# Vinmwaura/Quantized-Autoregression-Image-Generator

Hardware: AMD Instinct MI355X
Metric: image-tokens/sec at 1/2/4/8 GPUs; BMU argmin GB/s vs HBM peak (higher is better)
Workload: dtype f32; 1 GPU; BASELINE configs[1]: BMU (K=512; LR patch 32, HR patch 2) + base decoder-only Transformer train step, 32x32x4 latents (128x128 images), 257-token sequences, window 256; batch_per_gpu=64, global_batch=64, seq_len=256, in_dim=512, hidden_dim=2048, heads=64, dec_layers=7, enc_layers=0, params=78226440, parallelism=dp1, launch=eager stream launches

## Files before the change

include/qarig.h:

```cpp
#ifndef QARIG_H
#define QARIG_H

#include <stddef.h>
#include <stdint.h>

#ifdef __cplusplus
extern "C" {
#endif

#define QARIG_OK 0
#define QARIG_ERR_ARG -1
#define QARIG_ERR_LAUNCH -2
#define QARIG_ERR_WORKSPACE -3

#define QARIG_ACT_NONE 0
#define QARIG_ACT_SILU 1
#define QARIG_ACT_TANH 2
#define QARIG_ACT_SIGMOID 3

int qarig_version(void);
const char* qarig_target_arch(void);
int qarig_last_error(char* buf, size_t n);
int qarig_set_option(const char* name, int value);

// ... 150 lines not shown

int qarig_window_step_supported(int R, int window, int D, int H);

int qarig_window_assemble(const int64_t* ring, int64_t ldr, const int* ctl, int R, int W1, int Wp, int D,
                          int V, const float* table, const float* pe, int P, int pos_off, float* x,
                          int* rowmap, int* last_map, int* bad_flag, void* stream);

int qarig_window_attention(const float* q, const float* k, const float* v, int R, int H, int d, int n_keys,
                           int rows, int64_t batch_stride, const float* o_mul, int64_t ldmul, float* o,
                           void* stream);

int qarig_window_append(int* ctl, const int64_t* ids, int64_t* ring, int B, int64_t ldr, int* bad_flag,
                        void* stream);

size_t qarig_colsum_workspace_bytes(int M, int N);
int qarig_colsum_f32(const float* X, int64_t ldx, int M, int N, float* out, int accumulate,
                     void* workspace, size_t ws_bytes, void* stream);

int qarig_slab_reduce_rowsum_f32(const float* slabs, float* out, int64_t ldc, int M, int N, int nslab,
                                 int accumulate, const float* rs_part, float* rs_out, void* stream);


int qarig_patchify_fwd(const float* image, int N, int C, int H, int W, int pH, int pW,
                       float* patches, void* stream);
int qarig_unpatchify_fwd(const float* patches, int N, int C, int H, int W, int pH, int pW,
                         float* image, void* stream);

int qarig_codebook_gather_image(const int64_t* ids, int N, int C, int H, int W, int pH, int pW,
                                const float* codebook, int K, float* image, int* bad_flag,
                                void* stream);

int qarig_gather_rows(const int64_t* ids, int64_t R, int D, int K, const float* table, float* out,
                      int* bad_flag, void* stream);

int qarig_som_weights_fwd(const int64_t* bmu, int64_t R, int K, float two_var, float* g,
                          void* stream);

int qarig_som_band(const float* in, int K, int D, float two_var, int reach, float* out, void* stream);

int qarig_index_histogram(const int64_t* ids, int64_t n, int K, int64_t* counts, int* bad_flag,
                          void* stream);


int qarig_posemb_fwd(const float* pos, int R, int D, const float* freq, float* out, void* stream);

int qarig_assemble_tokens(const int64_t* lr, int S_lr, const int64_t* hr, int S_hr, int N, int base,
                          int k_lr, int k_hr, const int64_t* offs, int W, int64_t* hr_in,
                          int64_t* hr_tg, int64_t* pos, int* bad_flag, void* stream);

int qarig_embedding_fwd(const int64_t* ids, int M, int S, int D, int V, const float* table,
                        const float* pe, float* out, int* bad_flag, void* stream);
int qarig_embedding_bwd(const int64_t* ids, int M, int D, int V, const float* dy, float* dtable,
                        void* stream);

int qarig_layernorm_fwd(const float* x, int M, int D, float eps, const float* gamma,
                        const float* beta, const float* scale, const float* shift,
                        const int* mod_idx, float* y, float* mean, float* rstd, void* stream);
int qarig_layernorm_bwd(const float* dy, const float* x, const float* mean, const float* rstd,
                        const float* gamma, const float* scale, const int* mod_idx, int M, int D,
                        float* dx, float* dy_xhat, const float* dx_add, void* stream);

int qarig_rowmap_build(const int* idx, int M, int P, int* counts, int* offsets, int* rows,
                       int* bad_flag, void* stream);
int qarig_segment_sum(const float* src, const int* offsets, const int* rows, int P, int D,
                      float* out, void* stream);
int qarig_mul_rows_fwd(const float* a, const float* tab, const int* idx, float* y, int M, int D,
                       void* stream);
int qarig_mul_rows_bwd(const float* dy, const float* a, const float* tab, const int* idx, float* da,
                       float* db_tok, int M, int D, void* stream);
int qarig_layernorm_bwd_table(const float* dy, const float* x, const float* mean, const float* rstd,
                              const float* scale_tab, const int* offsets, const int* rows, int M, int P,
                              int D, float* dx, const float* dx_add, float* dscale, float* dshift,
                              void* stream);
int qarig_mul_rows_bwd_table(const float* dy, const float* a, const float* tab, const int* offsets,
                             const int* rows, int M, int P, int D, float* da, float* dg, void* stream);

int qarig_attention_fwd(const float* q, const float* k, const float* v, int N, int Sq, int Sk,
                        int H, int d, int causal, float sqrt_d, float* o, float* lse,
                        void* stream);
int qarig_attention_bwd(const float* q, const float* k, const float* v, const float* o,
                        const float* dO, const float* lse, int N, int Sq, int Sk, int H, int d,
                        int causal, float sqrt_d, float* dq, float* dk, float* dv, float* delta,
                        void* stream);

int qarig_attention_lp_fwd(const float* q, const float* k, const float* v, int N, int Sq, int Sk, int H,
                           int d, int causal, float sqrt_d, float* o, float* lse, void* stream);
int qarig_attention_lp_bwd(const float* q, const float* k, const float* v, const float* o,
                           const float* dO, const float* lse, int N, int Sq, int Sk, int H, int d,
                           int causal, float sqrt_d, float* dq, float* dk, float* dv, float* delta,
                           void* stream);

int qarig_attention_decode(const float* q, const float* k_new, const float* v_new, float* kcache,
                           float* vcache, int B, int H, int d, int len, const int* len_dev,
                           int max_len, int64_t batch_stride, float sqrt_d, const float* o_mul,
                           float* o, void* stream);

int qarig_cross_entropy_fwd(const float* logits, const int64_t* target, int M, int C, float* loss,
                            float* dlogits, float* row_ws, int* bad_flag, void* stream);
int qarig_cross_entropy_ld_fwd(const float* logits, int64_t ld_logits, const int64_t* target, int M, int C,
                               float* loss, float* dlogits, int64_t ld_dlogits, float* row_ws, int* bad_flag,
                               void* stream);

int qarig_cross_entropy_reg_fwd(const float* logits, const int64_t* target, int M, int C, float label_smoothing,
                                float z_loss, float* loss, float* dlogits, float* row_ws, int* bad_flag,
                                void* stream);

int qarig_token_score(const float* logits, const int64_t* target, int M, int C, int64_t ignore_index,
                      float* row_nll, int* row_rank, int* bad_flag, void* stream);
int qarig_score_reduce(const float* row_nll, const int* row_rank, int N, int S, int pos0, int P, int topk,
                       double* img_nll, double* pos_nll, int64_t* pos_cnt, int64_t* totals, void* stream);

size_t qarig_pair_error_workspace_bytes(int N, int64_t E);
int qarig_pair_error(const float* a, const float* b, int N, int64_t E, double* out, void* ws, size_t ws_bytes,
                     void* stream);
size_t qarig_ssim_workspace_bytes(int N, int C, int H, int W, int taps);
int qarig_ssim(const float* a, const float* b, int N, int C, int H, int W, const double* win, int taps, double c1,
               double c2, double* out, void* ws, size_t ws_bytes, void* stream);

size_t qarig_ssim_maps_bytes(int N, int C, int H, int W, int taps);
int qarig_ssim_fwd_maps(const float* a, const float* b, int N, int C, int H, int W, const double* win, int taps,
                        double c1, double c2, double* out, double* maps, void* ws, size_t ws_bytes, void* stream);
int qarig_ssim_bwd(const float* a, const float* b, const double* maps, const double* g, int N, int C, int H, int W,
                   const double* win, int taps, float* da, void* stream);

size_t qarig_mse_workspace_bytes(void);
int qarig_mse_fwd(const float* pred, const float* target, int64_t n, float* loss, float* dpred,
                  float* part_ws, void* stream);

int qarig_adam_step(float* p, const float* g, float* m, float* v, int64_t n, float beta1,
                    float beta2, float eps, float step_size, float bc2_sqrt, float grad_scale,
                    const float* dev_step, void* shadow_bf16, void* stream);

int qarig_adam_ema_step(float* p, const float* g, float* m, float* v, float* ema, int64_t n, float beta1,
                        float beta2, float eps, float step_size, float bc2_sqrt, float ema_w,
                        float grad_scale, const float* dev_step, void* shadow_bf16, void* stream);

int qarig_adamw_step(float* p, const float* g, float* m, float* v, float* ema, const unsigned char* decay_mask,
                     int64_t n, float beta1, float beta2, float eps, float step_size, float bc2_sqrt,
                     float ema_w, float decay, float grad_scale, const float* dev_step, void* shadow_bf16,
                     void* stream);

#define QARIG_GRAD_NORM_PARTIALS 2048
int qarig_grad_clip_coef(const float* g, int64_t n, float grad_scale, double max_norm, double* partials,
                         double* state, void* stream);
int qarig_adam_clip_step(float* p, const float* g, float* m, float* v, float* ema, const unsigned char* decay_mask,
                         int64_t n, float beta1, float beta2, float eps, float step_size, float bc2_sqrt,
                         float ema_w, float decay, float grad_scale, const float* dev_step, void* shadow_bf16,
                         const double* clip_state, void* stream);

int qarig_swap_f32(float* a, float* b, int64_t n, void* stream);

int qarig_mul_fwd(const float* a, const float* b, float* y, int64_t n, void* stream);
int qarig_mul_bwd(const float* dy, const float* a, const float* b, float* da, float* db, int64_t n,
                  void* stream);
int qarig_act_fwd(const float* x, float* y, int64_t n, int act, void* stream);
int qarig_act_bwd(const float* dy, const float* z, float* dz, int64_t n, int act, void* stream);
int qarig_scale_by(const float* x, const float* s, float* y, int64_t n, void* stream);

int qarig_dropout(const float* x, float* y, int64_t n, uint32_t threshold, float scale, uint32_t site,
                  const uint32_t* key, void* stream);


int qarig_conv2d_fwd(const float* x, int N, int Cin, int H, int W, const float* w,
                     const float* bias, int Cout, int k, int stride, int pad, int act, float* y,
                     float* preact, void* stream);
size_t qarig_conv2d_fwd_workspace_bytes(int Cin, int Cout, int k);
// ... 33 lines not shown
```

quantized-autoregression-image-generator_amd/csrc/attention.hip:

```cpp
#include <stdlib.h>

#include "qarig_common.h"

namespace qarig {

struct AttnDims {
    int N, Sq, Sk, H, causal;
    float c2;
    float rsd;
};

__device__ __forceinline__ float exp2_fast(float x) { return __builtin_amdgcn_exp2f(x); }

constexpr int HPB = 4;

__device__ __forceinline__ f32x4 mfma4(float a, float b, f32x4 c) {
    return __builtin_amdgcn_mfma_f32_4x4x1f32(a, b, c, 0, 0, 0);
}

typedef short s16x4 __attribute__((ext_vector_type(4)));
__device__ __forceinline__ uint32_t pack2_bf16(float a, float b) {
    typedef __bf16 bf16x2_t __attribute__((ext_vector_type(2)));
    typedef float f32x2_t __attribute__((ext_vector_type(2)));
    const f32x2_t f = {a, b};
// ... 442 lines not shown
        if (ibeg > c0) i0 = c0 + ((ibeg - c0) & ~7);
        for (; i0 < i1; i0 += 8) {
            const int ii = i0 - c0;
            f32x4 s0 = {0.f, 0.f, 0.f, 0.f}, s1 = s0, d0 = s0, d1 = s0;
            const T* qr = Qc + (ii + li) * Geo<HD>::RS;
            const T* gr = Gc + (ii + li) * Geo<HD>::RS;
            dot_rows<LP, HD>(s0, qr, kv);
            dot_rows<LP, HD>(s1, qr + 4 * Geo<HD>::RS, kv);
            dot_rows<LP, HD>(d0, gr, vv);
            dot_rows<LP, HD>(d1, gr + 4 * Geo<HD>::RS, vv);
            const f32x4 La = *reinterpret_cast<const f32x4*>(Lc + ii);
            const f32x4 Lb = *reinterpret_cast<const f32x4*>(Lc + ii + 4);
            const f32x4 Da = *reinterpret_cast<const f32x4*>(Dc + ii);
            const f32x4 Db = *reinterpret_cast<const f32x4*>(Dc + ii + 4);
            float p[8], ds[8];
#pragma unroll
            for (int r = 0; r < 4; ++r) {
                p[r] = exp2_fast(fmaf(s0[r], a.c2, -La[r]));
                p[4 + r] = exp2_fast(fmaf(s1[r], a.c2, -Lb[r]));
            }
            if (i0 + 8 > i1 || (a.causal && i0 < k0 + 63)) {
#pragma unroll
                for (int r = 0; r < 8; ++r)
                    if (i0 + r >= i1 || (a.causal && j > i0 + r)) p[r] = 0.0f;
            }
#pragma unroll
            for (int r = 0; r < 4; ++r) {
                ds[r] = p[r] * (d0[r] - Da[r]);
                ds[4 + r] = p[4 + r] * (d1[r] - Db[r]);
            }
            const Vals<LP> pa = make_vals<LP>(p[0], p[1], p[2], p[3]);
            const Vals<LP> pb = make_vals<LP>(p[4], p[5], p[6], p[7]);
            const Vals<LP> da = make_vals<LP>(ds[0], ds[1], ds[2], ds[3]);
            const Vals<LP> dbv = make_vals<LP>(ds[4], ds[5], ds[6], ds[7]);
#pragma unroll
            for (int g = 0; g < G; ++g) {
                const T* gt = GTc + (4 * g + li) * TS + ii;
                const T* qt = QTc + (4 * g + li) * TS + ii;
                if constexpr (LP) {
                    acc_cols<LP>(dva[g], gt, pa);
                    acc_cols<LP>(dka[g], qt, da);
                    acc_cols<LP>(dva[g], gt + 4, pb);
                    acc_cols<LP>(dka[g], qt + 4, dbv);
                } else {
                    const f32x4 ga = *reinterpret_cast<const f32x4*>(gt);
                    const f32x4 gb4 = *reinterpret_cast<const f32x4*>(gt + 4);
                    const f32x4 qa = *reinterpret_cast<const f32x4*>(qt);
                    const f32x4 qb4 = *reinterpret_cast<const f32x4*>(qt + 4);
#pragma unroll
                    for (int r = 0; r < 4; ++r) {
                        dva[g] = mfma4(ga[r], p[r], dva[g]);
                        dka[g] = mfma4(qa[r], ds[r], dka[g]);
                    }
#pragma unroll
                    for (int r = 0; r < 4; ++r) {
                        dva[g] = mfma4(gb4[r], p[4 + r], dva[g]);
                        dka[g] = mfma4(qb4[r], ds[4 + r], dka[g]);
                    }
                }
            }
        }
        if (t + 1 < nchunks) {
            T* nb = smem + ((t + 1) & 1) * BUF;
            chunk_store_rows<HD>(nb, rq);
            chunk_store_rows<HD>(nb + GOFF, rg);
            chunk_store_transposed<HD>(nb + QTOFF, TS, rq);
            chunk_store_transposed<HD>(nb + GTOFF, TS, rg);
            float* nl = ldbase + ((t + 1) & 1) * LDBUF;
            if (lth) { nl[threadIdx.x] = rl; nl[HPB * CH + threadIdx.x] = rd; }
        }
        __syncthreads();
    }
    if (active) {
#pragma unroll
        for (int g = 0; g < G; ++g) {
            *reinterpret_cast<float4*>(dk + roff + 4 * g) =
                make_float4(dka[g][0] * a.rsd, dka[g][1] * a.rsd, dka[g][2] * a.rsd, dka[g][3] * a.rsd);
            *reinterpret_cast<float4*>(dv + roff + 4 * g) =
                make_float4(dva[g][0], dva[g][1], dva[g][2], dva[g][3]);
        }
    }
}


}

using namespace qarig;

#define QARIG_HD_DISPATCH(d, ...)                                              \
    switch (d) {                                                                 \
        case 4: { constexpr int HD = 4; __VA_ARGS__; } break;                           \
        case 8: { constexpr int HD = 8; __VA_ARGS__; } break;                           \
        case 16: { constexpr int HD = 16; __VA_ARGS__; } break;                         \
        case 32: { constexpr int HD = 32; __VA_ARGS__; } break;                         \
        case 64: { constexpr int HD = 64; __VA_ARGS__; } break;                         \
        default:                                                                 \
            qarig_set_error("attention: head dim %d unsupported (4,8,16,32,64,128)", d); \
            return QARIG_ERR_ARG;                                                \
    }

int qarig_attention_wide_fwd(const float* q, const float* k, const float* v, int N, int Sq, int Sk, int H,
                             int causal, float sqrt_d, float* o, float* lse, hipStream_t st);
int qarig_attention_wide_bwd(const float* q, const float* k, const float* v, const float* o, const float* dO,
                             const float* lse, int N, int Sq, int Sk, int H, int causal, float sqrt_d, float* dq,
                             float* dk, float* dv, float* delta, hipStream_t st);
static int attn_wide_check(int N, int Sq, int Sk, int H, int causal) {
    QARIG_CHECK_ARG(N > 0 && Sq > 0 && Sk > 0 && H > 0, "attention: bad extents");
    QARIG_CHECK_DIMS("attention", N, Sq, H);
    QARIG_CHECK_DIMS("attention", N, Sk, H);
    QARIG_CHECK_ARG(H <= 65535 && N <= 65535, "attention (wide heads): more than 65535 heads or sequences");
    QARIG_CHECK_ARG(!causal || Sq == Sk, "attention: causal needs Sq == Sk (self-attention)");
    return QARIG_OK;
}

static int attn_check(int N, int Sq, int Sk, int H, int d, int causal) {
    QARIG_CHECK_ARG(N > 0 && Sq > 0 && Sk > 0 && H > 0 && d > 0, "attention: bad extents");
    QARIG_CHECK_DIMS("attention", N, Sq, H);
    QARIG_CHECK_DIMS("attention", N, Sk, H);
    QARIG_CHECK_ARG(d == 4 || d == 8 || d == 16 || d == 32 || d == 64,
                    "attention: head dim %d unsupported (4,8,16,32,64,128)", d);
    QARIG_CHECK_ARG((long long)N * ((H + 3) / 4) * ((Sq > Sk ? Sq : Sk) / 64 + 1) < (1LL << 31),
                    "attention: too many workgroups");
    QARIG_CHECK_ARG(!causal || Sq == Sk, "attention: causal needs Sq == Sk (self-attention)");
    return QARIG_OK;
}

static int attn_waves(int rows, int d, int option, int dflt, int wmax) {
    int w = option > 0 ? option : dflt;
    w = w >= 4 ? 4 : (w >= 2 ? 2 : 1);
    if (w > wmax) w = wmax;
    while (w > 1 && (w / 2) * 64 >= rows) w /= 2;
    while (w < wmax && (w * 256) / d < 8) w *= 2;
    return w;
}

#define QARIG_FWD_MAXT(HD) ((HD) <= 16 ? 1024 : 512)

template <typename K>
static int attn_set_lds(K kernel, size_t bytes, const char* what) {
    if (bytes > 160 * 1024) {
        qarig_set_error("%s: needs %zu B of LDS", what, bytes);
        return QARIG_ERR_ARG;
    }
    if (bytes > 48 * 1024) {
        hipError_t e = hipFuncSetAttribute(reinterpret_cast<const void*>(kernel),
                                           hipFuncAttributeMaxDynamicSharedMemorySize, (int)bytes);
        if (e != hipSuccess) {
            qarig_set_error("%s: hipFuncSetAttribute(%zu B LDS): %s", what, bytes, hipGetErrorString(e));
            return QARIG_ERR_LAUNCH;
        }
    }
    return QARIG_OK;
}

static size_t attn_lds_bytes(int threads, int d, int rows, int tr, bool ld, int lp) {
    const int W = HPB * d, CH = threads / (W / 4);
    const size_t img = 2 * (lp ? 2 : 4) * ((size_t)rows * CH * (W + 4) + (size_t)tr * W * (CH + 4));
    return ((img + 15) & ~(size_t)15) + (ld ? 2 * sizeof(float) * 2 * HPB * CH : 0);
}

template <bool LP>
static int attention_fwd_impl(const float* q, const float* k, const float* v, int N, int Sq, int Sk,
                              int H, int d, int causal, float sqrt_d, float* o, float* lse, void* stream) {
    QARIG_CHECK_ARG(q && k && v && o && lse, "attention_fwd: null pointer");
    if (d == 128) {
        if (int e = attn_wide_check(N, Sq, Sk, H, causal)) return e;
        QARIG_CHECK_ARG(sqrt_d > 0.0f, "attention: sqrt_d must be positive");
        return qarig_attention_wide_fwd(q, k, v, N, Sq, Sk, H, causal, sqrt_d, o, lse, (hipStream_t)stream);
    }
    if (int e = attn_check(N, Sq, Sk, H, d, causal)) return e;
    AttnDims a{N, Sq, Sk, H, causal, 1.4426950408889634f / sqrt_d, 1.0f / sqrt_d};
    const int W = attn_waves(Sq, d, g_qarig_opt.attn_qw, 2, d <= 16 ? 4 : 2);
    const int threads = 256 * W, rows = 64 * W;
    const size_t lds = attn_lds_bytes(threads, d, 1, 1, false, LP);
    dim3 grid((unsigned)(N * ((H + HPB - 1) / HPB) * ((Sq + rows - 1) / rows))), block(threads);
    QARIG_HD_DISPATCH(d, {
        auto kern = attn_fwd_kernel<HD, QARIG_FWD_MAXT(HD), LP>;
        if (int e = attn_set_lds(kern, lds, "attention_fwd")) return e;
        hipLaunchKernelGGL(kern, grid, block, lds, (hipStream_t)stream, q, k, v, a, o, lse);
    });
    QARIG_CHECK_LAUNCH("attention_fwd");
    return QARIG_OK;
}

template <bool LP>
static int attention_bwd_impl(const float* q, const float* k, const float* v, const float* o,
                              const float* dO, const float* lse, int N, int Sq, int Sk, int H, int d,
                              int causal, float sqrt_d, float* dq, float* dk, float* dv, float* delta,
                              void* stream) {
    QARIG_CHECK_ARG(q && k && v && o && dO && lse && dq && dk && dv && delta,
                    "attention_bwd: null pointer");
    if (d == 128) {
        if (int e = attn_wide_check(N, Sq, Sk, H, causal)) return e;
        QARIG_CHECK_ARG(sqrt_d > 0.0f, "attention: sqrt_d must be positive");
        return qarig_attention_wide_bwd(q, k, v, o, dO, lse, N, Sq, Sk, H, causal, sqrt_d, dq, dk, dv, delta,
                                        (hipStream_t)stream);
    }
    if (int e = attn_check(N, Sq, Sk, H, d, causal)) return e;
    AttnDims a{N, Sq, Sk, H, causal, 1.4426950408889634f / sqrt_d, 1.0f / sqrt_d};
    const int hgroups = (H + HPB - 1) / HPB;
    {
        const int W = attn_waves(Sq, d, g_qarig_opt.attn_bw, 2, 2);
        const int threads = 256 * W, rows = 64 * W;
        const size_t lds = attn_lds_bytes(threads, d, 2, 1, false, LP);
        dim3 grid((unsigned)(N * hgroups * ((Sq + rows - 1) / rows))), block(threads);
        QARIG_HD_DISPATCH(d, {
            auto kern = attn_bwd_dq_kernel<HD, 512, LP>;
            if (int e = attn_set_lds(kern, lds, "attention_bwd dq")) return e;
            hipLaunchKernelGGL(kern, grid, block, lds, (hipStream_t)stream, q, k, v, o, dO, lse, a, dq, delta);
        });
        QARIG_CHECK_LAUNCH("attention_bwd dq");
    }
    {
        const int W = attn_waves(Sk, d, g_qarig_opt.attn_bw, 2, 2);
        const int threads = 256 * W, rows = 64 * W;
        const size_t lds = attn_lds_bytes(threads, d, 2, 2, true, LP);
        dim3 grid((unsigned)(N * hgroups * ((Sk + rows - 1) / rows))), block(threads);
        QARIG_HD_DISPATCH(d, {
            auto kern = attn_bwd_dkv_kernel<HD, 512, LP>;
            if (int e = attn_set_lds(kern, lds, "attention_bwd dkv")) return e;
            hipLaunchKernelGGL(kern, grid, block, lds, (hipStream_t)stream, q, k, v, dO, lse, delta, a, dk, dv);
        });
        QARIG_CHECK_LAUNCH("attention_bwd dkv");
    }
    return QARIG_OK;
}

extern "C" int qarig_attention_fwd(const float* q, const float* k, const float* v, int N, int Sq,
                                   int Sk, int H, int d, int causal, float sqrt_d, float* o,
                                   float* lse, void* stream) {
    return attention_fwd_impl<false>(q, k, v, N, Sq, Sk, H, d, causal, sqrt_d, o, lse, stream);
}

extern "C" int qarig_attention_bwd(const float* q, const float* k, const float* v, const float* o,
                                   const float* dO, const float* lse, int N, int Sq, int Sk, int H,
                                   int d, int causal, float sqrt_d, float* dq, float* dk, float* dv,
                                   float* delta, void* stream) {
    return attention_bwd_impl<false>(q, k, v, o, dO, lse, N, Sq, Sk, H, d, causal, sqrt_d, dq, dk, dv,
                                     delta, stream);
}

extern "C" int qarig_attention_lp_fwd(const float* q, const float* k, const float* v, int N, int Sq,
                                      int Sk, int H, int d, int causal, float sqrt_d, float* o,
                                      float* lse, void* stream) {
    return attention_fwd_impl<true>(q, k, v, N, Sq, Sk, H, d, causal, sqrt_d, o, lse, stream);
}
extern "C" int qarig_attention_lp_bwd(const float* q, const float* k, const float* v, const float* o,
                                      const float* dO, const float* lse, int N, int Sq, int Sk, int H,
                                      int d, int causal, float sqrt_d, float* dq, float* dk, float* dv,
                                      float* delta, void* stream) {
    return attention_bwd_impl<true>(q, k, v, o, dO, lse, N, Sq, Sk, H, d, causal, sqrt_d, dq, dk, dv,
                                    delta, stream);
}

extern "C" int qarig_attention_decode(const float* q, const float* k_new, const float* v_new,
                                      float* kcache, float* vcache, int B, int H, int d, int len,
                                      const int* len_dev, int max_len, int64_t batch_stride,
                                      float sqrt_d, const float* o_mul, float* o, void* stream) {
    return qarig_decode_attention(q, k_new, v_new, kcache, vcache, B, H, d, len, len_dev, max_len, batch_stride, d,
                                  (int64_t)H * d, sqrt_d, o_mul, (int64_t)H * d, o, stream);
}
```

quantized-autoregression-image-generator_amd/csrc/capi.hip:

```cpp
#include <stdarg.h>
#include <stdio.h>
#include <string.h>

#include "qarig_common.h"

static thread_local char g_err[512] = "";

extern "C" void qarig_set_error(const char* fmt, ...) {
    va_list ap;
    va_start(ap, fmt);
    vsnprintf(g_err, sizeof(g_err), fmt, ap);
    va_end(ap);
}

extern "C" int qarig_version(void) { return 100; }

extern "C" int qarig_last_error(char* buf, size_t n) {
    if (!buf || n == 0) return QARIG_ERR_ARG;
    strncpy(buf, g_err, n - 1);
    buf[n - 1] = '\0';
    return QARIG_OK;
}

extern "C" const char* qarig_target_arch(void) { return "gfx950"; }

QarigOptions g_qarig_opt;

extern "C" int qarig_set_option(const char* name, int value) {
    struct Entry { const char* name; int* slot; };
    const Entry table[] = {
        {"gemm_dma", &g_qarig_opt.gemm_dma},       {"gemm_pair", &g_qarig_opt.gemm_pair},
        {"bmu_cs", &g_qarig_opt.bmu_cs},           {"bmu_groups", &g_qarig_opt.bmu_groups},
        {"bmu_coarse", &g_qarig_opt.bmu_coarse},   {"attn_qw", &g_qarig_opt.attn_qw},
        {"attn_bw", &g_qarig_opt.attn_bw},         {"lp_big", &g_qarig_opt.lp_big},
        {"lp_mfma16", &g_qarig_opt.lp_mfma16},     {"convt_pair", &g_qarig_opt.convt_pair},
        {"conv_ring", &g_qarig_opt.conv_ring},     {"gemm_xcd_splits", &g_qarig_opt.gemm_xcd_splits},
        {"decode_stream", &g_qarig_opt.decode_stream}, {"decode_rows", &g_qarig_opt.decode_rows},
        {"gemm_tile64", &g_qarig_opt.gemm_tile64}, {"gemm_x3", &g_qarig_opt.gemm_x3},
    };
    if (name)
        for (const Entry& e : table)
            if (strcmp(e.name, name) == 0) {
                const int old = *e.slot;
                *e.slot = value;
                return old;
            }
    qarig_set_error("set_option: unknown option %s (gemm_dma, gemm_pair, bmu_cs, bmu_groups, bmu_coarse, attn_qw, "
                    "attn_bw, lp_big, lp_mfma16, convt_pair, conv_ring, gemm_xcd_splits, decode_stream, decode_rows, gemm_tile64, gemm_x3)", name ? name : "(null)");
    return -2147483647 - 1;
}
```

quantized-autoregression-image-generator_amd/csrc/qarig_common.h:

```cpp
#pragma once
#include <hip/hip_runtime.h>
#include <stdint.h>

#define QARIG_OK 0
#define QARIG_ERR_ARG -1
#define QARIG_ERR_LAUNCH -2
#define QARIG_ERR_WORKSPACE -3

extern "C" void qarig_set_error(const char* fmt, ...);

extern "C" int qarig_gemm_tile64(int M, int N, int K);
extern "C" int qarig_decode_linear_supported(int M, int N, int K, int ln);
extern "C" int qarig_decode_linear_f32(const float* X, int64_t ldx, int64_t x_gs, float eps, const float* gamma,
                                       const float* beta, const float* scale, const float* shift, int64_t ldmod,
                                       const float* W, int64_t ldw, int64_t w_gs, const float* bias, int64_t bias_gs,
                                       const float* residual, int64_t ldr, const float* mul, int64_t ldmul, float* C,
                                       int64_t ldc, int64_t c_gs, int groups, int M, int N, int K, int act,
                                       void* stream);
extern "C" int qarig_decode_attention(const float* q, const float* k_new, const float* v_new, float* kcache,
                                      float* vcache, int B, int H, int d, int len, const int* len_dev, int max_len,
                                      int64_t batch_stride, int64_t head_stride, int64_t row_stride, float sqrt_d,
                                      const float* o_mul, int64_t ldmul, float* o, void* stream);

struct QarigOptions {
    int gemm_dma = 1;
    int gemm_xcd_splits = 1;
    int gemm_pair = -1;
    int bmu_cs = 0;
    int bmu_groups = -1;
    int bmu_coarse = -1;
    int attn_qw = 0;
    int attn_bw = 0;
    int lp_big = -1;
    int lp_mfma16 = 1;
    int convt_pair = 1;
    int gemm_x3 = 0;
    int gemm_tile64 = -1;
    int decode_rows = 1;
    int decode_stream = 1;
    int conv_ring = 1;
};
extern QarigOptions g_qarig_opt;

#define QARIG_CHECK_ARG(cond, ...)                 \
    do {                                           \
        if (!(cond)) {                             \
            qarig_set_error(__VA_ARGS__);          \
            return QARIG_ERR_ARG;                  \
        }                                          \
    } while (0)

#define QARIG_CHECK_LAUNCH(name)                                              \
    do {                                                                      \
        hipError_t e__ = hipGetLastError();                                   \
        if (e__ != hipSuccess) {                                              \
            qarig_set_error("%s: launch failed: %s", name, hipGetErrorString(e__)); \
            return QARIG_ERR_LAUNCH;                                          \
        }                                                                     \
    } while (0)

#include <initializer_list>
static inline bool qarig_dims_ok(std::initializer_list<long long> dims, long long max_each = 1LL << 24,
                                 long long max_prod = 1LL << 40) {
    long long p = 1;
    for (long long d : dims) {
        if (d < 1 || d > max_each) return false;
        if (p > max_prod / d) return false;
        p *= d;
    }
    return true;
}
#define QARIG_CHECK_DIMS(what, ...)                                                             \
    QARIG_CHECK_ARG(qarig_dims_ok({__VA_ARGS__}),                                               \
                    what ": extents must be positive, at most 2^24 each, product at most 2^40")

namespace qarig {

typedef float f32x16 __attribute__((ext_vector_type(16)));
typedef float f32x4 __attribute__((ext_vector_type(4)));

enum Act : int { ACT_NONE = 0, ACT_SILU = 1, ACT_TANH = 2, ACT_SIGMOID = 3 };

__device__ __forceinline__ float sigmoid_f(float x) {
    return __builtin_amdgcn_rcpf(1.0f + __builtin_amdgcn_exp2f(x * -1.4426950408889634f));
}

__device__ __forceinline__ float act_fwd(float x, int act) {
    switch (act) {
        case ACT_SILU: return x * sigmoid_f(x);
        case ACT_TANH: return tanhf(x);
        case ACT_SIGMOID: return sigmoid_f(x);
        default: return x;
    }
}

__device__ __forceinline__ float act_grad(float x, int act) {
    switch (act) {
        case ACT_SILU: {
            float s = sigmoid_f(x);
            return s * (1.0f + x * (1.0f - s));
        }
        case ACT_TANH: {
            float t = tanhf(x);
            return 1.0f - t * t;
        }
        case ACT_SIGMOID: {
            float s = sigmoid_f(x);
            return s * (1.0f - s);
        }
        default: return 1.0f;
    }
}

constexpr int BM = 128;
constexpr int BN = 128;
// ... 266 lines not shown
```

quantized-autoregression-image-generator_amd/qarig/_lib.py:

```python
import ctypes
import os
from ctypes import c_int, c_int64, c_size_t, c_void_p, c_float, c_char_p

import torch

_HERE = os.path.dirname(os.path.abspath(__file__))
LIB_PATH = os.path.join(os.path.dirname(_HERE), "lib",
                        os.environ.get("QARIG_LIB", "libqarig_hip.so"))

P = c_void_p
I = c_int
L = c_int64
Z = c_size_t
F = c_float
D = ctypes.c_double
U = ctypes.c_uint32

SIGNATURES = {
    "qarig_version": (I, []),
    "qarig_target_arch": (c_char_p, []),
    "qarig_last_error": (I, [c_char_p, Z]),
    "qarig_set_option": (I, [c_char_p, I]),
    "qarig_bmu_workspace_bytes": (Z, [L, I]),
    "qarig_bmu_fwd": (I, [P, I, I, I, I, I, I, P, I, I, P, P, Z, P]),
    "qarig_bmu_fwd_prepared": (I, [P, I, I, I, I, I, I, P, I, I, P, P, Z, P, P]),
    "qarig_bmu_fwd_coarse": (I, [P, I, I, I, I, I, I, P, I, I, P, P, P, P]),
    "qarig_bmu_coarse_workspace_bytes": (Z, [L, I]),
    "qarig_bmu_fwd_coarse_ws": (I, [P, I, I, I, I, I, I, P, I, I, P, P, P, P, Z, P]),
    "qarig_bmu_prepare_bytes": (Z, [I, I]),
    "qarig_bmu_prepare": (I, [P, I, I, P, P]),
    "qarig_gemm_ragged_tn": (I, [I, I, I]),
    "qarig_gemm_ragged_nt": (I, [I, I, I]),
    "qarig_gemm_workspace_bytes": (Z, [I, I, I]),
    "qarig_gemm_f32": (I, [P, L, I, P, L, I, P, L, I, I, I, P, P, L, P, L, I, P, L, I, I, I, P, P, Z,
                           P]),
    "qarig_gemm_tile64": (I, [I, I, I]),
    "qarig_gemm_x3_ok": (I, [I, I, I, I]),
    "qarig_gemm_grouped_supported": (I, [I, I, I, I]),
    "qarig_gemm_grouped_workspace_bytes": (Z, [I, I, I, I, I]),
    "qarig_gemm_f32_grouped": (I, [I, P, L, I, P, L, I, P, L, I, I, I, P, P, L, P, L, I, P, L, I, I, I, I, P,
                                   P, Z, P]),
    "qarig_gemm_f32_strided": (I, [P, L, P, L, L, P, L, L, P, L, I, I, I, I, I, P]),
    "qarig_gemm_lp_supported": (I, [I, I, I, I]),
    "qarig_gemm_lp_workspace_bytes": (Z, [I, I, I]),
    "qarig_gemm_lp": (I, [P, L, P, L, I, P, L, I, I, I, P, P, L, P, L, I, P, L, I, I, I, I, P, L, P, L, P, Z,
                          P]),
    "qarig_gemm_f8_supported": (I, [I, I, I]),
    "qarig_cast_fp8": (I, [P, L, P, P, P, P, P]),
    "qarig_gemm_f8": (I, [P, L, P, L, P, P, P, L, I, I, I, P, P, L, P, L, I, P, L, P, L, P]),
    "qarig_mx_quant_workspace_bytes": (Z, [I, I]),
    "qarig_mx_quant": (I, [P, L, I, I, I, P, P, P, P, P, I, P, Z, P]),
    "qarig_gemm_mx_supported": (I, [I, I, I, I]),
    "qarig_gemm_mx_workspace_bytes": (Z, [I, I, I]),
    "qarig_gemm_mx": (I, [P, L, P, L, P, L, P, L, P, L, I, I, I, P, P, L, P, L, I, P, L, I, I, I, I, P, L, P, L,
                          P, Z, P]),
    "qarig_cast_colsum_workspace_bytes": (Z, [I, I]),
    "qarig_cast_colsum": (I, [P, L, I, I, I, P, P, I, P, Z, P]),
    "qarig_cast_bf16": (I, [P, P, L, P]),
    "qarig_cast_transpose_bf16": (I, [P, L, I, I, P, P]),
    "qarig_colsum_workspace_bytes": (Z, [I, I]),
    "qarig_colsum_f32": (I, [P, L, I, I, P, I, P, Z, P]),
    "qarig_patchify_fwd": (I, [P, I, I, I, I, I, I, P, P]),
    "qarig_unpatchify_fwd": (I, [P, I, I, I, I, I, I, P, P]),
    "qarig_codebook_gather_image": (I, [P, I, I, I, I, I, I, P, I, P, P, P]),
    "qarig_gather_rows": (I, [P, L, I, I, P, P, P, P]),
    "qarig_som_weights_fwd": (I, [P, L, I, F, P, P]),
    "qarig_som_band": (I, [P, I, I, F, I, P, P]),
    "qarig_index_histogram": (I, [P, L, I, P, P, P]),
    "qarig_posemb_fwd": (I, [P, I, I, P, P, P]),
    "qarig_assemble_tokens": (I, [P, I, P, I, I, I, I, I, P, I, P, P, P, P, P]),
    "qarig_embedding_fwd": (I, [P, I, I, I, I, P, P, P, P, P]),
    "qarig_embedding_bwd": (I, [P, I, I, I, P, P, P]),
    "qarig_layernorm_fwd": (I, [P, I, I, F, P, P, P, P, P, P, P, P, P]),
    "qarig_layernorm_bwd": (I, [P, P, P, P, P, P, P, I, I, P, P, P, P]),
    "qarig_rowmap_build": (I, [P, I, I, P, P, P, P, P]),
    "qarig_segment_sum": (I, [P, P, P, I, I, P, P]),
    "qarig_mul_rows_fwd": (I, [P, P, P, P, I, I, P]),
    "qarig_mul_rows_bwd": (I, [P, P, P, P, P, P, I, I, P]),
    "qarig_layernorm_bwd_table": (I, [P, P, P, P, P, P, P, I, I, I, P, P, P, P, P]),
    "qarig_mul_rows_bwd_table": (I, [P, P, P, P, P, I, I, I, P, P, P]),
    "qarig_slab_reduce_rowsum_f32": (I, [P, P, L, I, I, I, I, P, P, P]),
    "qarig_attention_fwd": (I, [P, P, P, I, I, I, I, I, I, F, P, P, P]),
    "qarig_attention_lp_fwd": (I, [P, P, P, I, I, I, I, I, I, F, P, P, P]),
    "qarig_attention_lp_bwd": (I, [P, P, P, P, P, P, I, I, I, I, I, I, F, P, P, P, P, P]),
    "qarig_attention_decode": (I, [P, P, P, P, P, I, I, I, I, P, I, L, F, P, P, P]),
    "qarig_gemm_grouped_skinny_f32": (I, [P, L, L, P, L, L, P, L, L, P, L, I, I, I, I, I, P]),
    "qarig_gemm_skinny_ln_f32": (I, [P, L, F, P, P, P, P, L, P, L, L, P, L, L, P, L, P, L, I, I, I, I, I, P]),
    "qarig_decode_linear_supported": (I, [I, I, I, I]),
    "qarig_decode_linear_f32": (I, [P, L, L, F, P, P, P, P, L, P, L, L, P, L, P, L, P, L, P, L, L, I, I, I, I, I,
                                    P]),
    "qarig_decode_linear_bf16w": (I, [P, L, L, F, P, P, P, P, L, P, L, L, P, L, P, L, P, L, P, L, L, I, I, I, I, I,
                                      P]),
    "qarig_decode_embed": (I, [P, I, I, I, P, P, P, I, I, P, L, P, P, P, P]),
    "qarig_decode_attention_keys_per_pass": (ctypes.c_uint, [I]),
    "qarig_decode_attention": (I, [P, P, P, P, P, I, I, I, I, P, I, L, L, L, F, P, L, P, P]),
    "qarig_decode_sample": (I, [P, L, I, I, F, I, I, L, P, P, P, I, I, I, I, I, P, P, P, P, P]),
    "qarig_decode_sample_filtered": (I, [P, L, I, I, F, I, I, L, P, P, P, I, I, I, I, I, P, P, P, P, I, F, P]),
    "qarig_decode_decide": (I, [P, I, I, I, I, P, P, P, P, P, P]),
    "qarig_decode_rows": (I, [P, P, P, P, I, I, I, I, I, I, I, I, P]),
    "qarig_decode_cache_fill": (I, [P, P, L, L, P, I, I, I, I, I, I, P]),
    "qarig_decode_commit": (I, [P, I, I, I, P, P, L, P, P]),
    "qarig_decode_advance": (I, [P, I, P]),
    "qarig_window_step_supported": (I, [I, I, I, I]),
    "qarig_window_assemble": (I, [P, L, P, I, I, I, I, I, P, P, I, I, P, P, P, P, P]),
    "qarig_window_attention": (I, [P, P, P, I, I, I, I, I, L, P, L, P, P]),
    "qarig_window_append": (I, [P, P, P, I, L, P, P]),
    "qarig_attention_bwd": (I, [P, P, P, P, P, P, I, I, I, I, I, I, F, P, P, P, P, P]),
    "qarig_cross_entropy_fwd": (I, [P, P, I, I, P, P, P, P, P]),
    "qarig_cross_entropy_ld_fwd": (I, [P, L, P, I, I, P, P, L, P, P, P]),
    "qarig_cross_entropy_reg_fwd": (I, [P, P, I, I, F, F, P, P, P, P, P]),
    "qarig_token_score": (I, [P, P, I, I, L, P, P, P, P]),
    "qarig_score_reduce": (I, [P, P, I, I, I, I, I, P, P, P, P, P]),
    "qarig_pair_error_workspace_bytes": (Z, [I, L]),
    "qarig_pair_error": (I, [P, P, I, L, P, P, Z, P]),
    "qarig_ssim_workspace_bytes": (Z, [I, I, I, I, I]),
    "qarig_ssim": (I, [P, P, I, I, I, I, P, I, D, D, P, P, Z, P]),
    "qarig_ssim_maps_bytes": (Z, [I, I, I, I, I]),
    "qarig_ssim_fwd_maps": (I, [P, P, I, I, I, I, P, I, D, D, P, P, P, Z, P]),
    "qarig_ssim_bwd": (I, [P, P, P, P, I, I, I, I, P, I, P, P]),
    "qarig_mse_workspace_bytes": (Z, []),
    "qarig_mse_fwd": (I, [P, P, L, P, P, P, P]),
    "qarig_adam_step": (I, [P, P, P, P, L, F, F, F, F, F, F, P, P, P]),
    "qarig_adam_ema_step": (I, [P, P, P, P, P, L, F, F, F, F, F, F, F, P, P, P]),
    "qarig_adamw_step": (I, [P, P, P, P, P, P, L, F, F, F, F, F, F, F, F, P, P, P]),
    "qarig_grad_clip_coef": (I, [P, L, F, D, P, P, P]),
    "qarig_adam_clip_step": (I, [P, P, P, P, P, P, L, F, F, F, F, F, F, F, F, P, P, P, P]),
    "qarig_swap_f32": (I, [P, P, L, P]),
    "qarig_mul_fwd": (I, [P, P, P, L, P]),
    "qarig_mul_bwd": (I, [P, P, P, P, P, L, P]),
    "qarig_act_fwd": (I, [P, P, L, I, P]),
    "qarig_act_bwd": (I, [P, P, P, L, I, P]),
    "qarig_scale_by": (I, [P, P, P, L, P]),
    "qarig_dropout": (I, [P, P, L, U, F, U, P, P]),
    "qarig_conv2d_fwd": (I, [P, I, I, I, I, P, P, I, I, I, I, I, P, P, P]),
    "qarig_conv2d_fwd_workspace_bytes": (Z, [I, I, I]),
    "qarig_conv2d_fwd_workspace_bytes_n": (Z, [I, I, I, I, I, I, I]),
    "qarig_conv2d_fwd_ws": (I, [P, I, I, I, I, P, P, I, I, I, I, I, P, P, P, Z, I, P]),
    "qarig_conv_transpose2d_workspace_bytes": (Z, [I, I]),
    "qarig_conv_transpose2d_workspace_bytes_n": (Z, [I, I, I, I, I]),
    "qarig_conv_transpose2d_fwd": (I, [P, I, I, I, I, P, P, I, I, P, P, P, Z, I, P]),
    "qarig_conv2d_bwd_data_workspace_bytes": (Z, [I, I, I]),
    "qarig_conv2d_bwd_data_workspace_bytes_n": (Z, [I, I, I, I, I, I, I]),
    "qarig_conv_transpose2d_bwd_data_workspace_bytes_n": (Z, [I, I, I, I, I]),
    "qarig_conv2d_bwd_data": (I, [P, I, I, I, I, P, I, I, I, I, I, I, P, P, Z, P]),
    "qarig_conv_transpose2d_bwd_data": (I, [P, I, I, I, I, P, I, P, P]),
    "qarig_conv_transpose2d_bwd_data_ws": (I, [P, I, I, I, I, P, I, P, P, Z, P]),
    "qarig_conv_wgrad_workspace_bytes": (Z, [I, I, I]),
    "qarig_conv_wgrad": (I, [P, I, I, I, I, P, I, I, I, I, I, I, P, P, Z, P]),
    "qarig_conv_bias_grad": (I, [P, I, I, I, P, P]),
}

_lib = None


def load():
    global _lib
    if _lib is not None:
        return _lib
    if not os.path.exists(LIB_PATH):
        raise RuntimeError(
            f"{LIB_PATH} not found: build it with "
            "`python quantized-autoregression-image-generator_amd/build.py` "
            "(there is no CPU fallback for the qarig ops)")
    lib = ctypes.CDLL(LIB_PATH)
    for name, (res, args) in SIGNATURES.items():
        fn = getattr(lib, name)
        fn.restype = res
        fn.argtypes = args
    _lib = lib
    for name in OPTIONS:
        v = os.environ.get("QARIG_" + name.upper())
        if v is not None:
            lib.qarig_set_option(name.encode(), int(v))
            _option_values[name] = int(v)
    return lib


OPTIONS = ("gemm_dma", "gemm_pair", "bmu_cs", "bmu_groups", "bmu_coarse", "attn_qw", "attn_bw", "lp_big",
           "lp_mfma16", "convt_pair", "conv_ring", "gemm_xcd_splits", "decode_stream", "decode_rows", "gemm_tile64", "gemm_x3")


OPTION_EPOCH = 0


_option_values = {}


def set_option(name, value):
    global OPTION_EPOCH
    OPTION_EPOCH += 1
    old = load().qarig_set_option(name.encode(), int(value))
    if old == -2 ** 31:
        raise KeyError(f"{name}: {last_error()}")
    _option_values[name] = int(value)
    return old


def option_value(name):
    return _option_values.get(name)


def last_error():
    buf = ctypes.create_string_buffer(512)
    load().qarig_last_error(buf, 512)
    return buf.value.decode("utf-8", "replace")


N_CALLS = 0


def check(status, what):
    global N_CALLS
    N_CALLS += 1
    if status != 0:
        raise RuntimeError(f"{what} failed ({status}): {last_error()}")


def ptr(t):
    if t is None:
        return None
    return t.data_ptr()


_raw_stream = getattr(torch._C, "_cuda_getCurrentRawStream", None)


def stream():
    if _raw_stream is not None:
        return _raw_stream(torch.cuda.current_device())
    return torch.cuda.current_stream().cuda_stream


def require_cuda(*tensors):
    for t in tensors:
        if t is not None and not t.is_cuda:
            raise RuntimeError(
                "qarig ops run on MI355X only: got a CPU tensor "
                "(the CPU restatement lives in oracle/ and is test infrastructure)")


def f32c(t):
    if t.dtype != torch.float32:
        t = t.float()
    return t if t.is_contiguous() else t.contiguous()


_ws_cache = {}
_ws_retired = []


def workspace(nbytes, device, tag="default"):
    key = (device.index if device.index is not None else torch.cuda.current_device(), tag)
    buf = _ws_cache.get(key)
    if buf is None or buf.numel() < nbytes:
        if buf is not None:
            _ws_retired.append(buf)
        buf = torch.empty(max(int(nbytes), 1 << 20), dtype=torch.uint8, device=device)
        _ws_cache[key] = buf
    return buf
```

Before: 294,900 image-tokens/s.

## Add single-pass attention backward kernel for head dim 8 with LDS-accumulated dq

Adds a fused attention backward kernel for head dim 8 and sequences up to 256. Each block keeps dq accumulators for the whole sequence in LDS per wave and computes dk, dv and dq in one sweep over query chunks, replacing the previous multi-pass or multi-kernel backward. It is meant to cut redundant recomputation and global traffic for dq. The cost is a large LDS footprint, which may lower occupancy. A plan function and an option are added to gate the path.

```diff
diff --git a/include/qarig.h b/include/qarig.h
--- a/include/qarig.h
+++ b/include/qarig.h
@@ -256,6 +256,7 @@
                         const float* dO, const float* lse, int N, int Sq, int Sk, int H, int d,
                         int causal, float sqrt_d, float* dq, float* dk, float* dv, float* delta,
                         void* stream);
+int qarig_attention_bwd_plan(int Sq, int Sk, int H, int d, int causal, int lp);
 
 int qarig_attention_lp_fwd(const float* q, const float* k, const float* v, int N, int Sq, int Sk, int H,
                            int d, int causal, float sqrt_d, float* o, float* lse, void* stream);
diff --git a/quantized-autoregression-image-generator_amd/csrc/attention.hip b/quantized-autoregression-image-generator_amd/csrc/attention.hip
--- a/quantized-autoregression-image-generator_amd/csrc/attention.hip
+++ b/quantized-autoregression-image-generator_amd/csrc/attention.hip
@@ -548,6 +548,263 @@
     }
 }
 
+constexpr int ONEPASS_MAX_S = 256;
+constexpr int OP_ROUND = 16;
+constexpr int OP_TS = 64 + 4;
+constexpr int op_chunk(int kw) { return 32 * kw; }
+constexpr int op_shared(int kw) {
+    return 2 * op_chunk(kw) * (HPB * 8 + 4) + 2 * HPB * 8 * (op_chunk(kw) + 4) + 2 * HPB * op_chunk(kw);
+}
+constexpr int OP_WAVE = OP_ROUND * OP_TS + ONEPASS_MAX_S * 8;
+
+__device__ __forceinline__ void wave_lds_sync() {
+    __builtin_amdgcn_fence(__ATOMIC_RELEASE, "wavefront");
+    __builtin_amdgcn_wave_barrier();
+    __builtin_amdgcn_fence(__ATOMIC_ACQUIRE, "wavefront");
+}
+
+template <bool B> struct BoolC { static constexpr bool value = B; };
+
+template <int HD, int KW>
+__global__ __launch_bounds__(256 * KW, 2) void attn_bwd_onepass_kernel(
+    const float* __restrict__ q, const float* __restrict__ k, const float* __restrict__ v,
+    const float* __restrict__ o, const float* __restrict__ dO, const float* __restrict__ lse, AttnDims a,
+    float* __restrict__ dq, float* __restrict__ dk, float* __restrict__ dv) {
+    static_assert(HD == 8, "the lane = (key half, query, column group) mapping is that of two column groups");
+    static_assert(KW == 1 || KW == 2, "one or two waves per head");
+    extern __shared__ __attribute__((aligned(16))) unsigned char smem_raw[];
+    float* smem = reinterpret_cast<float*>(smem_raw);
+    constexpr int G = HD / 4;
+    constexpr int CH = op_chunk(KW), TS = CH + 4, RS = Geo<HD>::RS, W = Geo<HD>::W;
+    constexpr int GOFF = CH * RS, QTOFF = 2 * CH * RS, GTOFF = QTOFF + W * TS;
+    constexpr int LOFF = GTOFF + W * TS, DOFF = LOFF + HPB * CH;
+    constexpr int OP_SHARED = op_shared(KW);
+    static_assert(DOFF + HPB * CH == OP_SHARED, "LDS layout");
+    const int hgroups = (a.H + HPB - 1) / HPB;
+    const int hg = blockIdx.x % hgroups, n = blockIdx.x / hgroups;
+    const int lane = threadIdx.x & 63;
+    const int wave = __builtin_amdgcn_readfirstlane(threadIdx.x >> 6);
+    const int hh = wave & 3, kh = wave >> 2;
+    const int h = hg * HPB + hh;
+    const bool head_ok = h < a.H;
+    const int D = a.H * HD;
+    const int li = lane & 3;
+    const int cols_valid = (a.H - hg * HPB) * HD;
+    const int ks = lane >> 5, g2 = (lane >> 2) & 1, qrow = ((lane >> 3) & 3) * 4 + li;
+    float* tile = smem + OP_SHARED + wave * OP_WAVE;
+    float* accq = tile + OP_ROUND * OP_TS;
+#pragma unroll
+    for (int m = 0; m < ONEPASS_MAX_S * HD / 256; ++m)
+        *reinterpret_cast<f32x4*>(accq + (m * 64 + lane) * 4) = f32x4{0.f, 0.f, 0.f, 0.f};
+    const float* Qc = smem + hh * HD;
+    const float* Gc = smem + GOFF + hh * HD;
+    const float* QTc = smem + QTOFF + (hh * HD) * TS;
+    const float* GTc = smem + GTOFF + (hh * HD) * TS;
+    const float* Lc = smem + LOFF + hh * CH;
+    const float* Dc = smem + DOFF + hh * CH;
+
+    const float* qbase = q + (int64_t)n * a.Sq * D + hg * HPB * HD;
+    const float* gbase = dO + (int64_t)n * a.Sq * D + hg * HPB * HD;
+    const float* obase = o + (int64_t)n * a.Sq * D + hg * HPB * HD;
+    const float* lb = lse + ((int64_t)n * a.H + hg * HPB) * a.Sq;
+    const int lrow = threadIdx.x / CH, lcol = threadIdx.x - lrow * CH;
+    const bool lth = threadIdx.x < HPB * CH;
+    auto load_ld = [&](int c0, float& rl, float& rd) {
+        rl = 0.0f; rd = 0.0f;
+        if (lth && hg * HPB + lrow < a.H && c0 + lcol < a.Sq) {
+            rl = lb[(int64_t)lrow * a.Sq + c0 + lcol];
+            const int64_t ro = (int64_t)(c0 + lcol) * D + lrow * HD;
+#pragma unroll
+            for (int c = 0; c < HD; c += 4) {
+                const float4 tg = *reinterpret_cast<const float4*>(gbase + ro + c);
+                const float4 to = *reinterpret_cast<const float4*>(obase + ro + c);
+                rd = fmaf(tg.x, to.x, rd); rd = fmaf(tg.y, to.y, rd);
+                rd = fmaf(tg.z, to.z, rd); rd = fmaf(tg.w, to.w, rd);
+            }
+        }
+    };
+
+    const int nkg = (a.Sk + 63) >> 6;
+    const int nslots = KW == 1 ? nkg : (nkg > 2 ? 2 : 1);
+    for (int slot = 0; slot < nslots; ++slot) {
+        const int kg = KW == 1 ? slot : (slot == 0 ? kh : 3 - kh);
+        const bool part = kg < nkg;
+        const int k0 = kg * 64;
+        const int j = k0 + lane;
+        const bool active = part && head_ok && j < a.Sk;
+        const int64_t roff = ((int64_t)n * a.Sk + (active ? j : 0)) * D + h * HD;
+        Own<false, HD> kv, vv;
+        own_load<false, HD>(kv, k + roff, active);
+        own_load<false, HD>(vv, v + roff, active);
+        float kt[32];
+        wave_lds_sync();
+#pragma unroll
+        for (int c = 0; c < HD; ++c) tile[c * OP_TS + lane] = kv.f[c];
+        wave_lds_sync();
+#pragma unroll
+        for (int m = 0; m < 8; ++m) {
+            const f32x4 t4 = *reinterpret_cast<const f32x4*>(tile + (4 * g2 + li) * OP_TS + 32 * ks + 4 * m);
+            kt[4 * m] = t4[0]; kt[4 * m + 1] = t4[1]; kt[4 * m + 2] = t4[2]; kt[4 * m + 3] = t4[3];
+        }
+        wave_lds_sync();
+        f32x4 dka[G], dva[G];
+#pragma unroll
+        for (int g = 0; g < G; ++g) { dka[g] = f32x4{0.f, 0.f, 0.f, 0.f}; dva[g] = dka[g]; }
+
+        const int ibeg = !a.causal ? 0 : (KW == 1 ? k0 : 128 * slot);
+        const int nchunks = a.Sq > ibeg ? (a.Sq - ibeg + CH - 1) / CH : 0;
+        const int qlo = j >= a.Sk ? 0x7fffffff : (a.causal ? j : 0);
+
+        auto round = [&](int i0, int c0, int i1, auto edge_c) {
+            constexpr bool EDGE = decltype(edge_c)::value;
+#pragma unroll
+            for (int st = 0; st < OP_ROUND / 8; ++st) {
+                const int is = i0 + 8 * st, ii = is - c0;
+                const float* qr = Qc + (ii + li) * RS;
+                const float* gr = Gc + (ii + li) * RS;
+                f32x4 qa[G], qb[G], ga[G], gb[G];
+#pragma unroll
+                for (int g = 0; g < G; ++g) {
+                    qa[g] = *reinterpret_cast<const f32x4*>(qr + 4 * g);
+                    qb[g] = *reinterpret_cast<const f32x4*>(qr + 4 * RS + 4 * g);
+                    ga[g] = *reinterpret_cast<const f32x4*>(gr + 4 * g);
+                    gb[g] = *reinterpret_cast<const f32x4*>(gr + 4 * RS + 4 * g);
+                }
+                const f32x4 La = *reinterpret_cast<const f32x4*>(Lc + ii);
+                const f32x4 Lb = *reinterpret_cast<const f32x4*>(Lc + ii + 4);
+                const f32x4 Da = *reinterpret_cast<const f32x4*>(Dc + ii);
+                const f32x4 Db = *reinterpret_cast<const f32x4*>(Dc + ii + 4);
+                f32x4 gta[G], gtb[G], qta[G], qtb[G];
+#pragma unroll
+                for (int g = 0; g < G; ++g) {
+                    const float* gt = GTc + (4 * g + li) * TS + ii;
+                    const float* qt = QTc + (4 * g + li) * TS + ii;
+                    gta[g] = *reinterpret_cast<const f32x4*>(gt);
+                    gtb[g] = *reinterpret_cast<const f32x4*>(gt + 4);
+                    qta[g] = *reinterpret_cast<const f32x4*>(qt);
+                    qtb[g] = *reinterpret_cast<const f32x4*>(qt + 4);
+                }
+                f32x4 s0 = {0.f, 0.f, 0.f, 0.f}, s1 = s0, d0 = s0, d1 = s0;
+#pragma unroll
+                for (int g = 0; g < G; ++g)
+#pragma unroll
+                    for (int c = 0; c < 4; ++c) {
+                        s0 = mfma4(qa[g][c], kv.f[4 * g + c], s0);
+                        s1 = mfma4(qb[g][c], kv.f[4 * g + c], s1);
+                        d0 = mfma4(ga[g][c], vv.f[4 * g + c], d0);
+                        d1 = mfma4(gb[g][c], vv.f[4 * g + c], d1);
+                    }
+                float p[8], ds[8];
+#pragma unroll
+                for (int r = 0; r < 4; ++r) {
+                    p[r] = exp2_fast(fmaf(s0[r], a.c2, -La[r]));
+                    p[4 + r] = exp2_fast(fmaf(s1[r], a.c2, -Lb[r]));
+                }
+                if constexpr (EDGE) {
+#pragma unroll
+                    for (int r = 0; r < 8; ++r) {
+                        const bool keep = (is + r >= qlo) & (is + r < i1);
+                        p[r] = keep ? p[r] : 0.0f;
+                    }
+                }
+#pragma unroll
+                for (int r = 0; r < 4; ++r) {
+                    ds[r] = p[r] * (d0[r] - Da[r]);
+                    ds[4 + r] = p[4 + r] * (d1[r] - Db[r]);
+                }
+#pragma unroll
+                for (int r = 0; r < 8; ++r) tile[(8 * st + r) * OP_TS + lane] = ds[r];
+#pragma unroll
+                for (int r = 0; r < 4; ++r)
+#pragma unroll
+                    for (int g = 0; g < G; ++g) {
+                        dva[g] = mfma4(gta[g][r], p[r], dva[g]);
+                        dka[g] = mfma4(qta[g][r], ds[r], dka[g]);
+                    }
+#pragma unroll
+                for (int r = 0; r < 4; ++r)
+#pragma unroll
+                    for (int g = 0; g < G; ++g) {
+                        dva[g] = mfma4(gtb[g][r], p[4 + r], dva[g]);
+                        dka[g] = mfma4(qtb[g][r], ds[4 + r], dka[g]);
+                    }
+            }
+            wave_lds_sync();
+            float* ap = accq + (i0 + qrow) * HD + 4 * g2;
+            f32x4 acc0 = *reinterpret_cast<const f32x4*>(ap), acc1 = {0.f, 0.f, 0.f, 0.f};
+            if (ks != 0) acc0 = acc1;
+            const float* dr = tile + qrow * OP_TS + 32 * ks;
+            f32x4 d4[8];
+#pragma unroll
+            for (int m = 0; m < 8; ++m) d4[m] = *reinterpret_cast<const f32x4*>(dr + 4 * m);
+#pragma unroll
+            for (int m = 0; m < 4; ++m)
+#pragma unroll
+                for (int r = 0; r < 4; ++r) {
+                    acc0 = mfma4(kt[4 * m + r], d4[m][r], acc0);
+                    acc1 = mfma4(kt[16 + 4 * m + r], d4[4 + m][r], acc1);
+                }
+            wave_lds_sync();
+            f32x4 tot;
+#pragma unroll
+            for (int e = 0; e < 4; ++e) {
+                const float half = acc0[e] + acc1[e];
+                tot[e] = half + __shfl_xor(half, 32);
+            }
+            if (ks == 0) *reinterpret_cast<f32x4*>(ap) = tot;
+        };
+        float4 rq = make_float4(0.f, 0.f, 0.f, 0.f), rg = rq;
+        float rl = 0.0f, rd = 0.0f;
+        if (nchunks > 0) {
+            rq = chunk_load<HD>(qbase, D, ibeg, a.Sq, cols_valid);
+            rg = chunk_load<HD>(gbase, D, ibeg, a.Sq, cols_valid);
+            load_ld(ibeg, rl, rd);
+        }
+        for (int t = 0; t < nchunks; ++t) {
+            const int c0 = ibeg + t * CH;
+            __syncthreads();
+            chunk_store_rows<HD>(smem, rq);
+            chunk_store_rows<HD>(smem + GOFF, rg);
+            chunk_store_transposed<HD>(smem + QTOFF, TS, rq);
+            chunk_store_transposed<HD>(smem + GTOFF, TS, rg);
+            if (lth) { smem[LOFF + threadIdx.x] = rl; smem[DOFF + threadIdx.x] = rd; }
+            __syncthreads();
+            if (t + 1 < nchunks) {
+                rq = chunk_load<HD>(qbase, D, c0 + CH, a.Sq, cols_valid);
+                rg = chunk_load<HD>(gbase, D, c0 + CH, a.Sq, cols_valid);
+                load_ld(c0 + CH, rl, rd);
+            }
+            const int i1 = min(c0 + CH, a.Sq);
+            if (!part || (a.causal && c0 < k0)) continue;
+            for (int i0 = c0; i0 < i1; i0 += OP_ROUND) {
+                if (i0 + OP_ROUND > i1 || (a.causal && i0 < k0 + 63) || k0 + 64 > a.Sk)
+                    round(i0, c0, i1, BoolC<true>{});
+                else
+                    round(i0, c0, i1, BoolC<false>{});
+            }
+        }
+        if (active) {
+#pragma unroll
+            for (int g = 0; g < G; ++g) {
+                *reinterpret_cast<float4*>(dk + roff + 4 * g) =
+                    make_float4(dka[g][0] * a.rsd, dka[g][1] * a.rsd, dka[g][2] * a.rsd, dka[g][3] * a.rsd);
+                *reinterpret_cast<float4*>(dv + roff + 4 * g) =
+                    make_float4(dva[g][0], dva[g][1], dva[g][2], dva[g][3]);
+            }
+        }
+    }
+    __syncthreads();
+    const float* accs = smem + OP_SHARED + OP_ROUND * OP_TS;
+    for (int idx = threadIdx.x; idx < a.Sq * (HPB * G); idx += 256 * KW) {
+        const int qd = idx / (HPB * G), rem = idx - qd * (HPB * G);
+        const int hd = rem / G, g = rem - hd * G;
+        if (hg * HPB + hd >= a.H) continue;
+        f32x4 t4 = *reinterpret_cast<const f32x4*>(accs + hd * OP_WAVE + qd * HD + 4 * g);
+        if constexpr (KW == 2) t4 += *reinterpret_cast<const f32x4*>(accs + (HPB + hd) * OP_WAVE + qd * HD + 4 * g);
+        *reinterpret_cast<float4*>(dq + ((int64_t)n * a.Sq + qd) * D + (hg * HPB + hd) * HD + 4 * g) =
+            make_float4(t4[0] * a.rsd, t4[1] * a.rsd, t4[2] * a.rsd, t4[3] * a.rsd);
+    }
+}
 
 }
 
@@ -649,6 +906,13 @@
     return QARIG_OK;
 }
 
+extern "C" int qarig_attention_bwd_plan(int Sq, int Sk, int H, int d, int causal, int lp) {
+    if (g_qarig_opt.attn_onepass < 0 || lp || d != 8) return 0;
+    if (Sq < 1 || Sk < 1 || H < 1 || Sq > ONEPASS_MAX_S || Sk > ONEPASS_MAX_S) return 0;
+    if (causal && Sq != Sk) return 0;
+    return 1;
+}
+
 template <bool LP>
 static int attention_bwd_impl(const float* q, const float* k, const float* v, const float* o,
                               const float* dO, const float* lse, int N, int Sq, int Sk, int H, int d,
@@ -665,6 +929,25 @@
     if (int e = attn_check(N, Sq, Sk, H, d, causal)) return e;
     AttnDims a{N, Sq, Sk, H, causal, 1.4426950408889634f / sqrt_d, 1.0f / sqrt_d};
     const int hgroups = (H + HPB - 1) / HPB;
+    if (qarig_attention_bwd_plan(Sq, Sk, H, d, causal, LP)) {
+        const int kw = g_qarig_opt.attn_bw > 0 ? (g_qarig_opt.attn_bw >= 2 ? 2 : 1)
+                                               : ((long long)N * hgroups >= 512 ? 1 : 2);
+        if (kw == 2) {
+            const size_t lds = sizeof(float) * (op_shared(2) + 2 * HPB * OP_WAVE);
+            auto kern = attn_bwd_onepass_kernel<8, 2>;
+            if (int e = attn_set_lds(kern, lds, "attention_bwd onepass")) return e;
+            hipLaunchKernelGGL(kern, dim3((unsigned)(N * hgroups)), dim3(512), lds, (hipStream_t)stream, q, k, v, o,
+                               dO, lse, a, dq, dk, dv);
+        } else {
+            const size_t lds = sizeof(float) * (op_shared(1) + HPB * OP_WAVE);
+            auto kern = attn_bwd_onepass_kernel<8, 1>;
+            if (int e = attn_set_lds(kern, lds, "attention_bwd onepass")) return e;
+            hipLaunchKernelGGL(kern, dim3((unsigned)(N * hgroups)), dim3(256), lds, (hipStream_t)stream, q, k, v, o,
+                               dO, lse, a, dq, dk, dv);
+        }
+        QARIG_CHECK_LAUNCH("attention_bwd onepass");
+        return QARIG_OK;
+    }
     {
         const int W = attn_waves(Sq, d, g_qarig_opt.attn_bw, 2, 2);
         const int threads = 256 * W, rows = 64 * W;
diff --git a/quantized-autoregression-image-generator_amd/csrc/capi.hip b/quantized-autoregression-image-generator_amd/csrc/capi.hip
--- a/quantized-autoregression-image-generator_amd/csrc/capi.hip
+++ b/quantized-autoregression-image-generator_amd/csrc/capi.hip
@@ -37,6 +37,7 @@
         {"conv_ring", &g_qarig_opt.conv_ring},     {"gemm_xcd_splits", &g_qarig_opt.gemm_xcd_splits},
         {"decode_stream", &g_qarig_opt.decode_stream}, {"decode_rows", &g_qarig_opt.decode_rows},
         {"gemm_tile64", &g_qarig_opt.gemm_tile64}, {"gemm_x3", &g_qarig_opt.gemm_x3},
+        {"attn_onepass", &g_qarig_opt.attn_onepass},
     };
     if (name)
         for (const Entry& e : table)
@@ -46,6 +47,6 @@
                 return old;
             }
     qarig_set_error("set_option: unknown option %s (gemm_dma, gemm_pair, bmu_cs, bmu_groups, bmu_coarse, attn_qw, "
-                    "attn_bw, lp_big, lp_mfma16, convt_pair, conv_ring, gemm_xcd_splits, decode_stream, decode_rows, gemm_tile64, gemm_x3)", name ? name : "(null)");
+                    "attn_bw, lp_big, lp_mfma16, convt_pair, conv_ring, gemm_xcd_splits, decode_stream, decode_rows, gemm_tile64, gemm_x3, attn_onepass)", name ? name : "(null)");
     return -2147483647 - 1;
 }
diff --git a/quantized-autoregression-image-generator_amd/csrc/qarig_common.h b/quantized-autoregression-image-generator_amd/csrc/qarig_common.h
--- a/quantized-autoregression-image-generator_amd/csrc/qarig_common.h
+++ b/quantized-autoregression-image-generator_amd/csrc/qarig_common.h
@@ -31,6 +31,7 @@
     int bmu_coarse = -1;
     int attn_qw = 0;
     int attn_bw = 0;
+    int attn_onepass = 0;
     int lp_big = -1;
     int lp_mfma16 = 1;
     int convt_pair = 1;
diff --git a/quantized-autoregression-image-generator_amd/qarig/_lib.py b/quantized-autoregression-image-generator_amd/qarig/_lib.py
--- a/quantized-autoregression-image-generator_amd/qarig/_lib.py
+++ b/quantized-autoregression-image-generator_amd/qarig/_lib.py
@@ -106,7 +106,8 @@
     "qarig_window_attention": (I, [P, P, P, I, I, I, I, I, L, P, L, P, P]),
     "qarig_window_append": (I, [P, P, P, I, L, P, P]),
     "qarig_attention_bwd": (I, [P, P, P, P, P, P, I, I, I, I, I, I, F, P, P, P, P, P]),
-    "qarig_cross_entropy_fwd": (I, [P, P, I, I, P, P, P, P, P]),
+    "qarig_attention_bwd_plan": (I, [I, I, I, I, I, I]),
+    "qarig_cross_entropy_fwd":(I, [P, P, I, I, P, P, P, P, P]),
     "qarig_cross_entropy_ld_fwd": (I, [P, L, P, I, I, P, P, L, P, P, P]),
     "qarig_cross_entropy_reg_fwd": (I, [P, P, I, I, F, F, P, P, P, P, P]),
     "qarig_token_score": (I, [P, P, I, I, L, P, P, P, P]),
@@ -177,7 +178,8 @@
 
 
 OPTIONS = ("gemm_dma", "gemm_pair", "bmu_cs", "bmu_groups", "bmu_coarse", "attn_qw", "attn_bw", "lp_big",
-           "lp_mfma16", "convt_pair", "conv_ring", "gemm_xcd_splits", "decode_stream", "decode_rows", "gemm_tile64", "gemm_x3")
+           "lp_mfma16", "convt_pair", "conv_ring", "gemm_xcd_splits", "decode_stream", "decode_rows", "gemm_tile64", "gemm_x3",
+           "attn_onepass")
 
 
 OPTION_EPOCH = 0
```

Result: no change. 296,800 image-tokens/s (median of 6 runs) (+0.6%).
